# neozenith/sqlite-muninn

Measured on AMD Instinct MI355X. Metric: kNN queries/sec (10k-query batch, k=10, ef=128, 1M x 768 f32 HNSW index) + recall@10, higher is better.
Workload: dtype f32

## Files before the change

### include/muninn_hip.h

```cpp
#ifndef MUNINN_HIP_H
#define MUNINN_HIP_H

#include <stddef.h>
#include <stdint.h>

#ifdef __cplusplus
extern "C" {
#endif

#define MN_ABI_VERSION 2

typedef enum { MN_METRIC_L2 = 0, MN_METRIC_COSINE = 1, MN_METRIC_INNER_PRODUCT = 2 } mn_metric;

typedef enum { MN_ORDER_SSE = 0, MN_ORDER_WAVE = 1 } mn_order;

typedef enum {
    MN_BUILD_SEQUENTIAL = 0,
    MN_BUILD_BATCHED = 1
} mn_build_mode;

typedef struct {
    int64_t id;
    float distance;
} mn_search_result;
// ... 56 lines not shown

int mn_hnsw_slot_count(mn_index *idx);
int mn_hnsw_export_nodes(mn_index *idx, int64_t *ids, int *levels, int *deleted);
int mn_hnsw_export_vectors(mn_index *idx, float *out);
int mn_hnsw_row_width(mn_index *idx, int level);
int mn_hnsw_export_links(mn_index *idx, int level, int *out, int *width);

int64_t mn_hnsw_take_dirty(mn_index *idx, int64_t *ids, int64_t cap);

int64_t mn_hnsw_edges_of(mn_index *idx, const int64_t *ids, int n, int64_t *out_src, int64_t *out_dst, int *out_level,
                         float *out_dist, int64_t cap);

typedef struct {
    double last_kernel_ms;
    int64_t last_n_dist;
    int64_t last_n_expanded;
    int64_t last_n_overflow;
    int64_t last_n_exact_rows;
    int64_t last_n_rows_lanes4;
    int64_t last_n_rows_lanes8;
    int64_t last_n_rows_lanes16;
} mn_launch_stats;
int mn_hnsw_last_launch(mn_index *idx, mn_launch_stats *out);
typedef struct {
    double search_ms, link_ms;
    int64_t n_dist, n_expanded;
    int64_t batches, nodes;
} mn_build_stats;
int mn_hnsw_build_stats(mn_index *idx, mn_build_stats *out, int reset);
void *mn_dev_malloc(mn_index *idx, size_t bytes);
void mn_dev_free(mn_index *idx, void *p);
int mn_dev_upload(mn_index *idx, void *dst_dev, const void *src_host, size_t bytes);
int mn_dev_download(mn_index *idx, void *dst_host, const void *src_dev, size_t bytes);
int mn_hnsw_bruteforce_topk(mn_index *idx, const float *d_queries, int64_t nq, int k, int64_t *out_ids);

typedef struct {
    int64_t n_queries, n_mfma_queries, n_fallback_queries, n_rescored_rows, n_bound_violations;
    float kernel_ms;
} mn_exact_stats;
int mn_hnsw_search_exact_batch(mn_index *idx, const float *queries, int64_t nq, int k,
                               const int64_t *allow_ids, int64_t n_allow,
                               int64_t *out_ids, float *out_dists, int *out_counts);
int mn_hnsw_search_exact_batch_dev(mn_index *idx, const float *d_queries, int64_t nq, int k,
                                   const int64_t *allow_ids, int64_t n_allow,
                                   int64_t *d_out_ids, float *d_out_dists, int *d_out_counts);
int mn_hnsw_last_exact(mn_index *idx, mn_exact_stats *out);
// ... 176 lines not shown
```

### sqlite-muninn_amd/csrc/mn_beam.hpp

```cpp
#pragma once
#include "mn_dist.hpp"

template <bool COH> DEVI int ld_link(const int *p) {
    if (COH)
        return __hip_atomic_load(p, __ATOMIC_RELAXED, __HIP_MEMORY_SCOPE_AGENT);
    return *p;
}
DEVI void st_link(int *p, int v) { __hip_atomic_store(p, v, __ATOMIC_RELAXED, __HIP_MEMORY_SCOPE_AGENT); }


struct WHeap {
    uint2 *l;
    unsigned long long *g;
    int lcap, gcap;
    int size;
    int ovf;
    int sorted = 0;
};

DEVI uint2 hget(const WHeap &h, int i) {
    if (i < h.lcap)
        return h.l[i];
    unsigned long long v = __hip_atomic_load(&h.g[i - h.lcap], __ATOMIC_RELAXED, __HIP_MEMORY_SCOPE_AGENT);
    return make_uint2((unsigned)(v & 0xffffffffull), (unsigned)(v >> 32));
}
DEVI void hset(const WHeap &h, int i, uint2 v) {
    if (i < h.lcap)
        h.l[i] = v;
    else
        __hip_atomic_store(&h.g[i - h.lcap], (unsigned long long)v.x | ((unsigned long long)v.y << 32), __ATOMIC_RELAXED,
                           __HIP_MEMORY_SCOPE_AGENT);
}

DEVI void heap_push(WHeap &h, int slot, float d, int lane) {
    if (h.size + 1 >= h.lcap + h.gcap) {
        h.ovf = 1;
        return;
    }
    h.size++;
    const int idx = h.size;
    const int depth = 31 - __clz(idx);
    const bool anc = lane >= 1 && lane <= depth;
    const int p = anc ? (idx >> lane) : idx;
    const uint2 x = make_uint2(f2u(d), (unsigned)slot);
    uint2 it = x;
    if (anc)
        it = hget(h, p);
    unsigned long long stopm = __ballot(anc && (u2f(it.x) <= d));
    const int stop = stopm ? (__ffsll((long long)stopm) - 1) : depth + 1;
    if (lane >= 1 && lane < stop)
        hset(h, idx >> (lane - 1), it);
    if (lane == 0)
        hset(h, idx >> (stop - 1), x);
    __builtin_amdgcn_wave_barrier();
}

DEVI uint2 heap_pop(WHeap &h, int lane) {
    uint2 top = hget(h, 1);
    top.x = rflu(top.x);
    top.y = rflu(top.y);
    uint2 x = hget(h, h.size);
    x.x = rflu(x.x);
    x.y = rflu(x.y);
    h.size--;
    if (h.size > 0) {
        int idx = 1;
        const float xd = u2f(x.x);
        for (;;) {
            int left = 2 * idx;
            if (left > h.size)
                break;
            uint2 L, Rt;
            if (left + 1 < h.lcap) {
                uint4 c = *reinterpret_cast<const uint4 *>(&h.l[left]);
                L = make_uint2(c.x, c.y);
                Rt = make_uint2(c.z, c.w);
            } else {
                L = hget(h, left);
                Rt = (left + 1 <= h.size) ? hget(h, left + 1) : L;
            }
            L.x = rflu(L.x);
            L.y = rflu(L.y);
            Rt.x = rflu(Rt.x);
            Rt.y = rflu(Rt.y);
            int smallest = idx;
            float sd = xd;
            uint2 sv = x;
            if (u2f(L.x) < sd) {
                smallest = left;
                sd = u2f(L.x);
                sv = L;
            }
            if (left + 1 <= h.size && u2f(Rt.x) < sd) {
                smallest = left + 1;
                sv = Rt;
            }
            if (smallest == idx)
                break;
            if (lane == 0)
                hset(h, idx, sv);
            idx = smallest;
        }
        if (lane == 0)
            hset(h, idx, x);
    }
    __builtin_amdgcn_wave_barrier();
    return top;
}


struct CoopCtx {
    int *n;
    int *list;
    float *dist;
    float *qnorm;
    int nw, wv;
    float *tile = nullptr;
    int tile_rows = 0;
};

#define MN_PHASE_N 16
#ifdef MN_PHASE_TIMING
static __device__ unsigned long long mn_phase[MN_PHASE_N];
#define PH_DECL unsigned long long ph_t = __builtin_amdgcn_s_memrealtime()
#define PH_ADD(w, k)                                                                                                             \
    do {                                                                                                                         \
        const unsigned long long ph_n = __builtin_amdgcn_s_memrealtime();                                                        \
        (w).ph[k] += ph_n - ph_t;                                                                                                \
        ph_t = ph_n;                                                                                                             \
    } while (0)
#define PH_CNT(w, k, n) (w).ph[k] += (n)
#else
#define PH_DECL
#define PH_ADD(w, k)
#define PH_CNT(w, k, n)
#endif

struct WaveCtx {
#ifdef MN_PHASE_TIMING
    unsigned long long ph[MN_PHASE_N] = {0, 0, 0, 0, 0, 0, 0, 0, 0, 0, 0, 0, 0, 0, 0, 0};
#endif
    float *tile = nullptr;
    const float *q;
    float qnorm;
    int *scratch;
    unsigned long long n_dist, n_exp;
    int *rlog = nullptr;
    int rcap = 0, nr = 0;
    CoopCtx *coop = nullptr;
    int no_spec_rows = 0;
    int lp_on = 0;
    LoQuery lq = {0.0f, 0.0};
    unsigned long long n_skip = 0;
    int sv_lanes = 0;
    unsigned long long n_l8 = 0, n_l16 = 0;
};
DEVI bool getenv_spec_off(const WaveCtx &w) { return (w.no_spec_rows & 1) != 0; }

DEVI void log_row_read(const MnDevIndex &ix, WaveCtx &w, int node, int level, int lane) {
    if (!w.rlog)
        return;
    if (lane == 0 && w.nr < w.rcap) {
        int *e = w.rlog + (size_t)w.nr * MN_RLOG_INTS;
        e[0] = level == 0 ? node : -(ix.up_off[node] + level - 1) - 2;
        e[1] = (int)0xff800000u;
        e[2] = e[3] = -1;
        e[4] = 0;
    }
    w.nr++;
}
DEVI void log_greedy_detail(WaveCtx &w, float to_beat, int from, int moved_to, int lane) {
    if (!w.rlog)
        return;
    if (lane == 0 && w.nr >= 1 && w.nr <= w.rcap) {
        int *e = w.rlog + (size_t)(w.nr - 1) * MN_RLOG_INTS;
        e[1] = __float_as_int(to_beat);
        e[2] = from;
        e[3] = moved_to;
// ... 577 lines not shown
            return;
        w.n_dist = nd0;
        w.n_exp = ne0;
        w.nr = nr0;
        for (long long i = lane; i < bm_words; i += 64)
            bitmap[i] = 0u;
        __builtin_amdgcn_fence(__ATOMIC_RELEASE, "agent");
        __builtin_amdgcn_s_waitcnt(0);
        __builtin_amdgcn_wave_barrier();
    }
    res.sorted = 0;
    beam_layer<ORDER, NCH, COH, WIDE, LOG>(ix, w, cand, res, bitmap, entry, level, ef, lane);
}

DEVI uint2 res_take(WHeap &res, int i, int count, int lane) {
    if (res.sorted) {
        uint2 it = hget(res, count - i);
        it.x = rflu(it.x);
        it.y = rflu(it.y);
        return it;
    }
    return heap_pop(res, lane);
}
```

### sqlite-muninn_amd/csrc/mn_device.hpp

```cpp
#pragma once
#include <hip/hip_runtime.h>
#include <stdint.h>
#include <stdlib.h>

#define MN_WAVE 64

typedef unsigned mn_lo_t;
#define MN_LO_BITS 10
#define MN_LO_CMAX 511
#define MN_LO_LINE_CODES 96
#define MN_LO_LINE_WORDS 32
struct __align__(16) MnLoMeta {
    float scale;
    float resid;
    float xn_lo;
    float xn_hi;
};
#define MN_LO_MIN_LD 192
__host__ __device__ inline bool mn_lo_enabled(int ld) { return ld >= MN_LO_MIN_LD && (ld & 63) == 0; }
__host__ __device__ inline int mn_lo_lines(int ld) { return (ld + MN_LO_LINE_CODES - 1) / MN_LO_LINE_CODES; }
__host__ __device__ inline size_t mn_lo_row_words(int ld) { return (size_t)mn_lo_lines(ld) * MN_LO_LINE_WORDS; }
__host__ __device__ inline int mn_lo_q_floats(int ld) { return mn_lo_enabled(ld) ? mn_lo_lines(ld) * MN_LO_LINE_CODES : ld; }
__host__ __device__ inline int mn_lo_code(unsigned w, int f) { return (int)(w << (32 - MN_LO_BITS * (f + 1))) >> (32 - MN_LO_BITS); }
__host__ __device__ inline unsigned mn_lo_pack(int c0, int c1, int c2) {
// ... 3 lines not shown
constexpr int MN_ORDER_WAVE_V = 1;

struct MnDevIndex {
    const float *vectors;
    const float *norms;
    int *links0;
    int *links_up;
    const int *up_off;
    const signed char *levels;
    const unsigned char *deleted;
    unsigned char *dirty;
    const long long *ids;
    int dim, ld, metric, order;
    int W0, WU;
    int M0, MU;
    int WX;
    int n_slots;
    int n_pool_rows;
    int has_deleted;
    const mn_lo_t *vec_lo;
    const MnLoMeta *lo_meta;
};

#define MN_QC 6
struct MnSearchArgs {
    const float *queries;
    const int *query_slots;
    long long nq;
    int k;
    int ef;
    int entry_slot, max_level;
    long long *out_ids;
    float *out_dists;
    int *out_counts;
    int *sel;
    int *nsel;
    int nlev;
    const int *up_bm_index;
    unsigned *bitmap0;
    long long bm0_words;
    unsigned *bitmap_up;
    long long bmu_words;
    uint2 *cand_ovf;
    int cand_gcap;
    uint2 *res_ovf;
    int res_gcap;
    unsigned long long *counters;
    unsigned long long *q_counters;
    int use_tile;
    int lds_bitmap;
    int *readlog;
    int readcap;
    int *nread;
    int lat_tile_rows;
    unsigned lat_tile_off;
    int surv_lanes;
    int no_spec_rows;
};
size_t mn_lds_optin_limit();
bool mn_lds_grant(const void *kernel, size_t bytes);
template <typename K> inline bool mn_lds_grant_for(K kernel, size_t bytes) { return mn_lds_grant(reinterpret_cast<const void *>(kernel), bytes); }
inline int mn_no_spec_rows(long long n_slots, int ld) {
    const char *sr = getenv("MN_SPEC_ROWS");
    const bool big = (size_t)n_slots * ld * sizeof(float) > ((size_t)256 << 20);
    return sr ? (atoi(sr) == 0 ? 1 : 0) : (big ? 0 : 1);
}

#ifndef MN_CAND_LDS
#define MN_CAND_LDS 256
#endif
#ifndef MN_RES_LDS
#define MN_RES_LDS 256
#endif

void mn_module_touch_kernels();
void mn_module_touch_seq();
void mn_module_touch_spec();
void mn_module_touch_build();
void mn_launch_prep_rows(const MnDevIndex &ix, int first_slot, int n, float *norms_out, mn_lo_t *lo_out, MnLoMeta *meta_out,
                         hipStream_t st);
int mn_launch_dist_batch(int metric, int order, const float *d_query, const float *d_rows, long long n, int dim, int ld,
// ... 79 lines not shown
```

### sqlite-muninn_amd/csrc/mn_index.hip

```cpp
#include "mn_index_int.hpp"

#include <cmath>
#include <cstdarg>
#include <cstdio>
#include <unordered_map>
#include <mutex>

#define MN_MAX_M 512
#define MN_MAX_ROW 2048

static thread_local std::string g_err;

void set_err(const char *fmt, ...) {
    va_list ap;
    va_start(ap, fmt);
    mn_vformat(g_err, fmt, ap);
    va_end(ap);
}

#include <atomic>
static std::atomic<long long> g_alloc_count{0}, g_alloc_fail_at{0};
static inline void *mn_counted_alloc(size_t n) {
    const long long c = g_alloc_count.fetch_add(1, std::memory_order_relaxed) + 1;
    if (c == g_alloc_fail_at.load(std::memory_order_relaxed))
// ... 940 lines not shown
            }
            ne++;
        }
    return ne;
} MN_GUARD_END(set_err, MN_NOTHING, -1)


extern "C" int mn_hnsw_build_stats(mn_index *x, mn_build_stats *out, int reset) try {
    *out = x->bstats;
    if (reset)
        x->bstats = {0, 0, 0, 0, 0, 0};
    return 0;
} MN_GUARD_END(set_err, MN_NOTHING, -1)

extern "C" int mn_hnsw_last_launch(mn_index *x, mn_launch_stats *out) try {
    if (use_device(x))
        return -1;
    if (!x->last_on_host && fetch_counters(x))
        return -1;
    *out = x->last;
    return 0;
} MN_GUARD_END(set_err, MN_NOTHING, -1)

extern "C" void *mn_dev_malloc(mn_index *x, size_t bytes) try {
    void *p = nullptr;
    if (hipSetDevice(x->device) != hipSuccess || hipMalloc(&p, bytes) != hipSuccess) {
        set_err("mn_dev_malloc(%zu) failed", bytes);
        return nullptr;
    }
    return p;
} MN_GUARD_END(set_err, MN_NOTHING, nullptr)
extern "C" void mn_dev_free(mn_index *x, void *p) {
    (void)hipSetDevice(x->device);
    (void)hipFree(p);
}
extern "C" int mn_dev_upload(mn_index *x, void *dst, const void *src, size_t bytes) try {
    if (use_device(x))
        return -1;
    HIPCHK(hipMemcpy(dst, src, bytes, hipMemcpyHostToDevice));
    return 0;
} MN_GUARD_END(set_err, MN_NOTHING, -1)
extern "C" int mn_dev_download(mn_index *x, void *dst, const void *src, size_t bytes) try {
    if (use_device(x))
        return -1;
    HIPCHK(hipStreamSynchronize(x->stream));
    HIPCHK(hipMemcpy(dst, src, bytes, hipMemcpyDeviceToHost));
// ... 3 lines not shown
```

### sqlite-muninn_amd/csrc/mn_index_int.hpp

```cpp
#pragma once
#include "../../include/muninn_hip.h"
#include "mn_comm.hpp"
#include "mn_device.hpp"
#include "mn_guard.hpp"
#include "mn_host.hpp"

#include <algorithm>
#include <cstdlib>
#include <cstring>
#include <string>
#include <vector>

void set_err(const char *fmt, ...) __attribute__((format(printf, 1, 2)));
#define HIPCHK(expr) MN_HIPCHK(set_err, expr)

template <typename T> struct DevBuf {
    T *p = nullptr;
    size_t cap = 0;
    DevBuf() = default;
    DevBuf(const DevBuf &) = delete;
    DevBuf &operator=(const DevBuf &) = delete;
    ~DevBuf() { release(); }
    int reserve(size_t n, bool keep, hipStream_t st, int fill_byte = -1, size_t want = 0) {
        if (n <= cap)
// ... 81 lines not shown
    DevBuf<unsigned long long> ws_counters;
    DevBuf<int> ws_state;
    DevBuf<int> er_slot, er_level, er_nbr;
    DevBuf<float> er_dist;
    DevBuf<int> ws_readlog, ws_nread, ws_ncommit, d_stamp0, d_stampU, d_sidx0, d_sidxU, d_saved_rows, d_pre_act, d_pre_cnt, d_pre_row, d_spec_why;
    int spec_epoch = 0;
    std::vector<int> staged;
    DevBuf<int> d_staged;
    DevBuf<int> sh_sel, sh_nsel, sh_gcnt;
    DevBuf<int> ws_chlog;
    bool want_chlog = false;
    std::vector<int> h_chlog;
    std::vector<unsigned char> h_stale;
    int n_stale = 0;
    unsigned char *pin = nullptr;
    size_t pin_cap = 0;
    DevBuf<unsigned long long> sh_ovf;
    int sh_ovf_pending = 0;
    DevBuf<long long> sh_gids;
    DevBuf<float> sh_gd;
    long long last_spec_searched = 0;
    bool broken = false;
    mn_launch_stats last = {0, 0, 0, 0, 0, 0, 0, 0};
    mn_exact_stats last_exact = {0, 0, 0, 0, 0, 0.0f};
};

int use_device(mn_index *x);
MnDevIndex dev_view(mn_index *x);
int ht_find(const mn_index *x, int64_t id);
void ht_grow(mn_index *x);
int random_level(mn_index *x);
int host_add_node(mn_index *x, int64_t id, int level, int deleted);
int64_t first_table_full(const mn_index *x, int64_t n);
void mark_stale(mn_index *x, int slot);
struct InsertUndo {
    int first, node_count, max_level, n_pool_rows, old_cap = 0, grew_at = -1;
    unsigned rng;
    int64_t entry_id;
    std::vector<int> old_ht;
};
void undo_insert(mn_index *x, InsertUndo &u);
int sync_meta(mn_index *x);
int upload_vectors(mn_index *x, int first, const float *vecs, int n, bool src_on_device = false);
int pull_links(mn_index *x);
int push_links(mn_index *x);
unsigned char *pin_reserve(mn_index *x, size_t need);
// ... 20 lines not shown
```

### sqlite-muninn_amd/csrc/mn_index_search.hip

```cpp
#include "mn_index_int.hpp"

#include <cstdio>


static int reserve_search_ws(mn_index *x, int64_t nq, int ef) {
    hipStream_t st = x->stream;
    if (x->ws_bm0.reserve((size_t)nq * bm0_words(x->n_slots), false, st)) return -1;
    if (x->ws_cand.reserve((size_t)nq * cand_gcap(ef), false, st)) return -1;
    if (x->ws_res.reserve((size_t)nq * res_gcap(ef), false, st)) return -1;
    if (x->ws_counters.reserve(8, false, st)) return -1;
    return 0;
}

int prepare_search_ws(mn_index *x, int64_t nq, int ef, MnSearchArgs &a, bool zero_counters, bool lds_bitmap_ok) {
    hipStream_t st = x->stream;
    a.bm0_words = bm0_words(x->n_slots);
    a.cand_gcap = cand_gcap(ef);
    a.res_gcap = res_gcap(ef);
    if (reserve_search_ws(x, nq, ef))
        return -1;
    a.lds_bitmap = lds_bitmap_ok && nq <= 128 &&
                   (long long)mn_search_lds_bytes(x->ld, true) + 1024 + a.bm0_words * (long long)sizeof(unsigned) <= 64 * 1024 &&
                   !(getenv("MN_COOP") && atoi(getenv("MN_COOP")) == 0) && !(getenv("MN_LDS_BITMAP") && atoi(getenv("MN_LDS_BITMAP")) == 0);
    if (!a.lds_bitmap)
        HIPCHK(hipMemsetAsync(x->ws_bm0.p, 0, (size_t)nq * a.bm0_words * sizeof(unsigned), st));
    if (zero_counters)
        HIPCHK(hipMemsetAsync(x->ws_counters.p, 0, 8 * sizeof(unsigned long long), st));
    a.bitmap0 = x->ws_bm0.p;
    a.cand_ovf = x->ws_cand.p;
    a.res_ovf = x->ws_res.p;
    a.counters = x->ws_counters.p;
    a.bitmap_up = nullptr;
    a.bmu_words = 0;
    a.no_spec_rows = mn_no_spec_rows(x->n_slots, x->ld);
#ifdef MN_SSE_TILE_PATH
    const char *e = getenv("MN_SSE_TILE");
    a.use_tile = e ? atoi(e) : 1;
#else
    a.use_tile = 0;
#endif
    return 0;
}

void last_from_counters(mn_index *x, const unsigned long long *c, bool timed) {
    float ms = 0;
    if (!timed)
        x->last.last_kernel_ms = 0.0f;
    else if (hipEventElapsedTime(&ms, x->ev0, x->ev1) == hipSuccess)
        x->last.last_kernel_ms = ms;
    x->last.last_n_dist = (int64_t)c[0];
    x->last.last_n_expanded = (int64_t)c[1];
    x->last.last_n_overflow = (int64_t)c[2];
    x->last.last_n_exact_rows = (int64_t)(c[0] - c[3]);
    x->last.last_n_rows_lanes8 = (int64_t)c[4];
    x->last.last_n_rows_lanes16 = (int64_t)c[5];
    x->last.last_n_rows_lanes4 = x->last.last_n_exact_rows - (int64_t)(c[4] + c[5]);
}

int fetch_counters(mn_index *x) {
    unsigned long long c[8];
    if (!x->ws_counters.p)
        return 0;
    HIPCHK(hipMemcpyAsync(c, x->ws_counters.p, sizeof(c), hipMemcpyDeviceToHost, x->stream));
    HIPCHK(hipStreamSynchronize(x->stream));
    last_from_counters(x, c, true);
    return 0;
}

static int search_batch_dev_impl(mn_index *x, const float *d_queries, int64_t nq, int k, int ef, int64_t *d_ids, float *d_dists,
                                 int *d_counts, unsigned long long *q_counters) {
    if (use_device(x))
        return -1;
    if (nq <= 0)
        return 0;
    if (k <= 0) {
        set_err("mn_hnsw_search: k must be > 0");
        return -1;
    }
    if (ef < k)
        ef = k;
    hipStream_t st = x->stream;
    if (x->entry_id == -1 || x->node_count == 0) {
        HIPCHK(hipMemsetAsync(d_counts, 0, (size_t)nq * sizeof(int), st));
        HIPCHK(hipMemsetAsync(d_ids, 0xFF, (size_t)nq * k * sizeof(int64_t), st));
        HIPCHK(hipMemsetAsync(d_dists, 0, (size_t)nq * k * sizeof(float), st));
        return 0;
    }
    if (push_links(x) || sync_meta(x))
// ... 79 lines not shown
    hipStream_t st = x->stream;
    const size_t qb = (size_t)nq * x->dim * sizeof(float), ib = (size_t)nq * k * sizeof(int64_t), db = (size_t)nq * k * sizeof(float);
    const size_t cb = ((size_t)nq * sizeof(int) + 7) & ~(size_t)7;
    const size_t o_ids = (qb + 15) & ~(size_t)15, o_d = o_ids + ib, o_c = (o_d + db + 7) & ~(size_t)7, o_cnt = o_c + cb;
    const size_t need = o_cnt + (size_t)nq * MN_QC * sizeof(unsigned long long);
    if (push_links(x) || sync_meta(x))
        return -1;
    if (!pin_reserve(x, need)) {
        set_err("mn_hnsw_search: cannot allocate %zu bytes of pinned host memory", need);
        return -1;
    }
    HIPCHK(hipStreamSynchronize(st));
    memcpy(x->pin, queries, qb);
    unsigned long long *qc = reinterpret_cast<unsigned long long *>(x->pin + o_cnt);
    if (search_batch_dev_impl(x, (const float *)x->pin, nq, k, ef, (int64_t *)(x->pin + o_ids), (float *)(x->pin + o_d),
                              (int *)(x->pin + o_c), qc))
        return -1;
    const bool launched = x->entry_id != -1 && x->node_count > 0;
    HIPCHK(hipStreamSynchronize(st));
    memcpy(out_ids, x->pin + o_ids, ib);
    memcpy(out_dists, x->pin + o_d, db);
    memcpy(out_counts, x->pin + o_c, (size_t)nq * sizeof(int));
    if (launched) {
        unsigned long long tot[MN_QC] = {0, 0, 0, 0, 0, 0};
        for (int64_t q = 0; q < nq; q++)
            for (int i = 0; i < MN_QC; i++)
                tot[i] += qc[q * MN_QC + i];
        last_from_counters(x, tot, false);
        x->last_on_host = true;
        if (x->last.last_n_overflow) {
            set_err("mn_hnsw_search: %lld queries exceeded heap workspace", (long long)x->last.last_n_overflow);
            return -1;
        }
    }
    return 0;
}

template <typename F>
static int with_staged_io(mn_index *x, const float *queries, size_t nq, int k, int64_t *out_ids, float *out_dists, int *out_counts,
                          F &&dev_face) {
    hipStream_t st = x->stream;
    if (queries && x->ws_q.reserve(nq * x->dim, false, st)) return -1;
    if (x->ws_outi.reserve(nq * k, false, st)) return -1;
    if (x->ws_outd.reserve(nq * k, false, st)) return -1;
    if (x->ws_outc.reserve(nq, false, st)) return -1;
    if (queries)
        HIPCHK(hipMemcpyAsync(x->ws_q.p, queries, nq * x->dim * sizeof(float), hipMemcpyHostToDevice, st));
    if (dev_face())
        return -1;
    HIPCHK(hipMemcpyAsync(out_ids, x->ws_outi.p, nq * k * sizeof(int64_t), hipMemcpyDeviceToHost, st));
    HIPCHK(hipMemcpyAsync(out_dists, x->ws_outd.p, nq * k * sizeof(float), hipMemcpyDeviceToHost, st));
// ... 347 lines not shown
```

### sqlite-muninn_amd/csrc/mn_kernels.hip

```cpp
#include "mn_device.hpp"
#include <cstdio>
#include <cstdlib>
#include <mutex>
#include <unordered_map>

#include "mn_dist.hpp"
#include "mn_dispatch.hpp"


DEVI double wave_sum_f64(double v) {
#pragma unroll
    for (int m = 32; m >= 1; m >>= 1)
        v += __shfl_xor(v, m);
    return v;
}

template <int ORDER>
__global__ void __launch_bounds__(64)
    k_prep_rows(MnDevIndex ix, int first_slot, int n, float *norms_out, mn_lo_t *lo_out, MnLoMeta *meta_out) {
    extern __shared__ float lds[];
    const int lane = threadIdx.x;
    int slot = first_slot + blockIdx.x;
    if (blockIdx.x >= n)
        return;
    const float *row = ix.vectors + (size_t)slot * ix.ld;
// ... 191 lines not shown
        w.lq.qs_lo = rfl_f64(w.lq.qs_lo);
        w.lq.qn_hi = rfl_f64(w.lq.qn_hi);
        w.qnorm = u2f(rflu(f2u(w.qnorm)));
        w.sv_lanes = a.surv_lanes;
    }
    if (BUILD && a.readlog) {
        w.rlog = a.readlog + (size_t)qi * a.readcap * MN_RLOG_INTS;
        w.rcap = a.readcap;
    }

    WHeap cand, res;
    cand.l = cand_l;
    cand.lcap = MN_CAND_LDS;
    cand.g = reinterpret_cast<unsigned long long *>(a.cand_ovf + (size_t)qi * a.cand_gcap);
    cand.gcap = a.cand_gcap;
    cand.size = 0;
    cand.ovf = 0;
    res.l = res_l;
    res.lcap = MN_RES_LDS;
    res.g = reinterpret_cast<unsigned long long *>(a.res_ovf + (size_t)qi * a.res_gcap);
    res.gcap = a.res_gcap;
    res.size = 0;
    res.ovf = 0;

    unsigned *bm0 = lds_bitmap ? lds_bitmap : a.bitmap0 + (size_t)qi * a.bm0_words;
    int cur = a.entry_slot;

    if (!BUILD) {
        for (int l = a.max_level; l > 0; l--)
            cur = greedy_layer<ORDER, NCH, false, WIDE>(ix, w, cur, l, lane);
        if (LAT)
            beam_layer_auto<ORDER, NCH, false, WIDE>(ix, w, cand, res, bm0, a.bm0_words, cur, 0, a.ef, lane);
        else
            beam_layer<ORDER, NCH, false, WIDE, false, LP>(ix, w, cand, res, bm0, cur, 0, a.ef, lane);
        int count = res.size;
        int outn = count < a.k ? count : a.k;
        for (int i = count - 1; i >= 0; i--) {
            uint2 it = res_take(res, i, count, lane);
            if (i < a.k && lane == 0) {
                a.out_ids[qi * a.k + i] = ix.ids[it.y];
                a.out_dists[qi * a.k + i] = -u2f(it.x);
            }
        }
        if (lane == 0) {
            for (int i = outn; i < a.k; i++) {
                a.out_ids[qi * a.k + i] = -1;
                a.out_dists[qi * a.k + i] = 0.0f;
            }
            a.out_counts[qi] = outn;
        }
    } else {
        const int level = ix.levels[qslot];
        for (int l = a.max_level; l > level; l--)
            cur = greedy_layer<ORDER, NCH, false, WIDE, LAT>(ix, w, cur, l, lane);
        int start = level < a.max_level ? level : a.max_level;
        for (int l = start; l >= 0; l--) {
            unsigned *bm = bm0;
            if (l > 0)
                bm = a.bitmap_up + ((size_t)a.up_bm_index[qi] * a.max_level + (l - 1)) * a.bmu_words;
            if (LAT)
                beam_layer_auto<ORDER, NCH, false, WIDE, true>(ix, w, cand, res, bm, l > 0 ? a.bmu_words : a.bm0_words, cur, l, a.ef, lane);
            else
                beam_layer<ORDER, NCH, false, WIDE>(ix, w, cand, res, bm, cur, l, a.ef, lane);
            const int M_max = (l == 0) ? ix.M0 : ix.MU;
            int count = res.size;
            int keep = count < M_max ? count : M_max;
            int *sel = a.sel + ((size_t)qi * a.nlev + l) * ix.M0;
            int first = cur;
            for (int i = count - 1; i >= 0; i--) {
                uint2 it = res_take(res, i, count, lane);
                if (i < keep && lane == 0)
                    sel[i] = (int)it.y;
                if (i == 0)
                    first = (int)it.y;
            }
            if (lane == 0)
                a.nsel[qi * a.nlev + l] = keep;
            if (count > 0)
                cur = first;
        }
    }
    if (lane == 0) {
        if (BUILD && a.readlog)
            a.nread[qi] = LAT ? w.nr : a.readcap + 1;
        if (a.q_counters) {
            a.q_counters[(size_t)qi * MN_QC + 0] = w.n_dist;
            a.q_counters[(size_t)qi * MN_QC + 1] = w.n_exp;
            a.q_counters[(size_t)qi * MN_QC + 2] = (cand.ovf || res.ovf) ? 1ull : 0ull;
            a.q_counters[(size_t)qi * MN_QC + 3] = w.n_skip;
            a.q_counters[(size_t)qi * MN_QC + 4] = w.n_l8;
            a.q_counters[(size_t)qi * MN_QC + 5] = w.n_l16;
        } else {
            atomicAdd(&a.counters[0], w.n_dist);
            atomicAdd(&a.counters[1], w.n_exp);
            if (cand.ovf || res.ovf)
                atomicAdd(&a.counters[2], 1ull);
            if (LP && w.n_skip)
                atomicAdd(&a.counters[3], w.n_skip);
            if (LP && w.n_l8)
                atomicAdd(&a.counters[4], w.n_l8);
            if (LP && w.n_l16)
                atomicAdd(&a.counters[5], w.n_l16);
        }
    }
}

template <int ORDER, int NCH, bool BUILD, bool WIDE = false, bool LP = false>
__global__ void __launch_bounds__(64) k_beam(MnDevIndex ix, MnSearchArgs a) {
    extern __shared__ __align__(16) unsigned char smem[];
    if ((long long)blockIdx.x >= a.nq)
        return;
    beam_query<ORDER, NCH, BUILD, WIDE, false, LP>(ix, a, blockIdx.x, threadIdx.x, smem, nullptr);
}

#define MN_COOP_WAVES 8
// ... 132 lines not shown
    const char *lp = getenv("MN_LOWPREC_FILTER");
    if (!build && ix.vec_lo && ix.lo_meta && !(lp && atoi(lp) == 0)) {
        MnSearchArgs al = a;
        const char *sv = getenv("MN_SURVIVOR_LANES");
        const int svl = sv ? atoi(sv) : 0;
        al.surv_lanes = (svl == 4 || svl == 8 || svl == 16) ? svl : 0;
        if (wide)
            hipLaunchKernelGGL((k_beam<ORDER, NCH, false, true, true>), grid, block, lds, st, ix, al);
        else
            hipLaunchKernelGGL((k_beam<ORDER, NCH, false, false, true>), grid, block, lds, st, ix, al);
        return;
    }
    if (wide) {
        if (build)
            hipLaunchKernelGGL((k_beam<ORDER, NCH, true, true>), grid, block, lds, st, ix, a);
        else
            hipLaunchKernelGGL((k_beam<ORDER, NCH, false, true>), grid, block, lds, st, ix, a);
    } else if (build)
        hipLaunchKernelGGL((k_beam<ORDER, NCH, true>), grid, block, lds, st, ix, a);
    else
        hipLaunchKernelGGL((k_beam<ORDER, NCH, false>), grid, block, lds, st, ix, a);
}

int mn_launch_search(const MnDevIndex &ix, const MnSearchArgs &a, bool build, hipStream_t st) {
    if (a.nq <= 0)
        return 0;
    if (ix.order == MN_ORDER_SSE_V) {
        const char *qe = getenv("MN_SSE_QUAD");
        if (MN_SSE_QUAD2 > 0 && (ix.dim >> 4) >= MN_SSE_QUAD2 && !(qe && atoi(qe) == 0))
            launch_beam<MN_ORDER_SSE_V, 1>(ix, a, build, st);
        else
            launch_beam<MN_ORDER_SSE_V, 0>(ix, a, build, st);
        return 0;
    }
    mn_for_wave_walk(ix.ld, [&](auto O, auto N) { launch_beam<O(), N()>(ix, a, build, st); });
    return 0;
}


template <int ORDER, int NCH>
__global__ void __launch_bounds__(64)
    k_edge_rows(MnDevIndex ix, const int *row_slot, const int *row_level, int n_rows, int *out_nbr, float *out_dist) {
    extern __shared__ __align__(16) unsigned char smem[];
    const int lane = threadIdx.x;
    const int r = blockIdx.x;
    if (r >= n_rows)
        return;
    float *q = reinterpret_cast<float *>(smem);
    const int s = row_slot[r], level = row_level[r];
// ... 96 lines not shown
```

### sqlite-muninn_amd/csrc/mn_seq.hip

```cpp
#include "mn_beam.hpp"
#include "mn_prune.hpp"
#include "mn_dispatch.hpp"

struct MnSeqArgs {
    const int *slots;
    int n;
    int ef;
    int *state;
    unsigned *bitmap0;
    long long bm0_words;
    unsigned *bitmap_up;
    long long bmu_words;
    uint2 *cand_ovf;
    int cand_gcap;
    uint2 *res_ovf;
    int res_gcap;
    unsigned long long *counters;
    int SB;
    int LW;
    int *chlog;
    int chcap;
    int pre_rows, pre_w;
    int wave_floats, lat_tile_rows;
    int no_spec_rows;
};
#define MN_CH_INTS 5

DEVI void seq_log(const MnSeqArgs &a, int &nlog, int op, int src, int level, int dst, unsigned dist_bits) {
    if (nlog < 0)
        return;
    if (nlog >= a.chcap) {
        nlog = -1;
        return;
    }
    int *e = a.chlog + 1 + (size_t)nlog * MN_CH_INTS;
    e[0] = op;
    e[1] = src;
    e[2] = level;
    e[3] = dst;
    e[4] = (int)dist_bits;
    nlog++;
}

DEVI int *seq_row(const MnDevIndex &ix, int node, int level) {
    if (level == 0)
        return ix.links0 + (size_t)node * ix.W0;
    return ix.links_up + ((size_t)ix.up_off[node] + (level - 1)) * ix.WU;
// ... 93 lines not shown
    if (coop.wv != 0) {
        seq_helper<ORDER, NCH>(ix, a, q, coop, selbuf, pre_nd, pre_cnt, tvw, lane);
        return;
    }

    WaveCtx w;
    w.coop = &coop;
    w.no_spec_rows = a.no_spec_rows;
    w.q = q;
    w.scratch = scratch;
    w.n_dist = 0;
    w.n_exp = 0;
    WHeap cand, res;
    cand.l = cand_l;
    cand.lcap = MN_CAND_LDS;
    cand.g = reinterpret_cast<unsigned long long *>(a.cand_ovf);
    cand.gcap = a.cand_gcap;
    cand.size = 0;
    cand.ovf = 0;
    res.l = res_l;
    res.lcap = MN_RES_LDS;
    res.g = reinterpret_cast<unsigned long long *>(a.res_ovf);
    res.gcap = a.res_gcap;
    res.size = 0;
    res.ovf = 0;

    int entry = a.state[0];
    int maxl = a.state[1];
    int nlog = a.chlog ? 0 : -1;

    for (int it = 0; it < a.n; it++) {
        const int s = a.slots[it];
        const int level = ix.levels[s];
        const float *sv = ix.vectors + (size_t)s * ix.ld;
        __builtin_amdgcn_wave_barrier();
        for (int i = lane; i < ix.ld; i += 64)
            q[i] = sv[i];
        __builtin_amdgcn_s_waitcnt(0);
        __builtin_amdgcn_wave_barrier();
        w.qnorm = ix.metric == 1 ? ix.norms[s] : 0.0f;
        if (lane == 0)
            *coop.qnorm = w.qnorm;

        int cur = entry;
        for (int l = maxl; l > level; l--)
            cur = greedy_layer<ORDER, NCH, true, WIDE>(ix, w, cur, l, lane);
// ... 170 lines not shown
    a.state = d_state;
    a.bitmap0 = bitmap0;
    a.bm0_words = bm0_words;
    a.bitmap_up = bitmap_up;
    a.bmu_words = bmu_words;
    a.cand_ovf = cand_ovf;
    a.cand_gcap = cand_gcap;
    a.res_ovf = res_ovf;
    a.res_gcap = res_gcap;
    a.counters = counters;
    a.SB = (ix.M0 + 63) & ~63;
    a.LW = (ix.WX + 1 + 63) & ~63;
    if (a.LW < 192)
        a.LW = 192;
    size_t lds = mn_insert_seq_lds_bytes(ix);
    const size_t base = lds - MN_SEQ_COOP_BYTES;
    int pre_rows = 0, pre_w = 0;
    size_t pre = seq_pre_bytes(ix, &pre_rows, &pre_w);
    const char *pe = getenv("MN_SEQ_PRE");
    if (pe && atoi(pe) == 0)
        pre = 0;
    a.pre_rows = a.pre_w = a.wave_floats = a.lat_tile_rows = 0;
    a.no_spec_rows = mn_no_spec_rows(ix.n_slots, ix.ld);
    const size_t lds0 = lds;
    const char *te = getenv("MN_LAT_TILE");
    for (int rows = ix.order == MN_ORDER_SSE_V && ix.ld >= 256 && !(te && atoi(te) == 0) ? 4 : 0; rows >= 0; rows = rows == 4 ? 2 : rows == 2 ? 0 : -1) {
        const int wf = std::max(pre ? ix.ld : 0, rows ? mn_lat_tile_floats(ix.ld, rows) : 0);
        const size_t need = lds0 + pre + (size_t)MN_SEQ_WAVES * wf * sizeof(float);
        if (rows == 0 && !pre)
            break;
        if (need <= (rows ? mn_lds_optin_limit() : (size_t)MN_LDS_LIMIT)) {
            lds = need;
            a.wave_floats = wf;
            a.lat_tile_rows = rows;
            if (pre) {
                a.pre_rows = pre_rows;
                a.pre_w = pre_w;
            }
            break;
        }
    }
    const char *co = getenv("MN_COOP");
    const dim3 blk(co && atoi(co) == 0 ? 64 : MN_SEQ_WAVES * 64);
    mn_for_row_walk(ix.order, ix.ld, [&](auto O, auto N) {
        if (lds > 64 * 1024) {
            const void *kp = ix.WX > 64 ? reinterpret_cast<const void *>(k_insert_seq<O(), N(), true>)
// ... 40 lines not shown
```

### sqlite-muninn_amd/hnsw.py

```python
from __future__ import annotations

import ctypes as C
import os

import numpy as np

from .build import LIB

METRIC = {"l2": 0, "cosine": 1, "inner_product": 2}
ORDER_SSE, ORDER_WAVE = 0, 1
BUILD_SEQUENTIAL, BUILD_BATCHED = 0, 1

_f32p = np.ctypeslib.ndpointer(np.float32, flags="C_CONTIGUOUS")
_i64p = np.ctypeslib.ndpointer(np.int64, flags="C_CONTIGUOUS")
_i32p = np.ctypeslib.ndpointer(np.int32, flags="C_CONTIGUOUS")


class MuninnHipError(RuntimeError):
    pass


class _Result(C.Structure):
    _fields_ = [("id", C.c_int64), ("distance", C.c_float)]

# ... 63 lines not shown
    ("mn_hnsw_delete", C.c_int, [C.c_void_p, C.c_int64]),
    ("mn_hnsw_get_vector", C.c_int, [C.c_void_p, C.c_int64, _f32p]),
    ("mn_hnsw_node_count", C.c_int, [C.c_void_p]),
    ("mn_hnsw_entry_point", C.c_int64, [C.c_void_p]),
    ("mn_hnsw_max_level", C.c_int, [C.c_void_p]),
    ("mn_hnsw_node_level", C.c_int, [C.c_void_p, C.c_int64]),
    ("mn_hnsw_node_deleted", C.c_int, [C.c_void_p, C.c_int64]),
    ("mn_hnsw_neighbors", C.c_int, [C.c_void_p, C.c_int64, C.c_int, _i64p, C.c_int]),
    ("mn_hnsw_load_node", C.c_int, [C.c_void_p, C.c_int64, _f32p, C.c_int, C.c_int]),
    ("mn_hnsw_load_neighbors", C.c_int, [C.c_void_p, C.c_int64, C.c_int, _i64p, C.c_int]),
    ("mn_hnsw_set_entry", C.c_int, [C.c_void_p, C.c_int64, C.c_int]),
    ("mn_hnsw_slot_count", C.c_int, [C.c_void_p]),
    ("mn_hnsw_export_nodes", C.c_int, [C.c_void_p, _i64p, _i32p, _i32p]),
    ("mn_hnsw_export_vectors", C.c_int, [C.c_void_p, _f32p]),
    ("mn_hnsw_export_links", C.c_int, [C.c_void_p, C.c_int, _i32p, C.POINTER(C.c_int)]),
    ("mn_hnsw_row_width", C.c_int, [C.c_void_p, C.c_int]),
    ("mn_hnsw_batch_stage", C.c_int, [C.c_void_p, _i64p, _f32p, C.c_int64]),
    ("mn_hnsw_batch_dims", C.c_int, [C.c_void_p, C.POINTER(C.c_int), C.POINTER(C.c_int)]),
    ("mn_hnsw_batch_search", C.c_int, [C.c_void_p, C.c_int, C.c_int, C.c_void_p, C.c_void_p]),
    ("mn_hnsw_batch_link", C.c_int, [C.c_void_p, C.c_void_p, C.c_void_p]),
    ("mn_hnsw_take_dirty", C.c_int64, [C.c_void_p, _i64p, C.c_int64]),
    ("mn_hnsw_edges_of", C.c_int64, [C.c_void_p, _i64p, C.c_int, _i64p, _i64p, _i32p, _f32p, C.c_int64]),
    ("mn_hnsw_last_launch", C.c_int, [C.c_void_p, C.POINTER(LaunchStats)]),
    ("mn_hnsw_build_stats", C.c_int, [C.c_void_p, C.POINTER(BuildStats), C.c_int]),
    ("mn_dev_malloc", C.c_void_p, [C.c_void_p, C.c_size_t]),
    ("mn_dev_free", None, [C.c_void_p, C.c_void_p]),
    ("mn_dev_upload", C.c_int, [C.c_void_p, C.c_void_p, C.c_void_p, C.c_size_t]),
    ("mn_dev_download", C.c_int, [C.c_void_p, C.c_void_p, C.c_void_p, C.c_size_t]),
    ("mn_hnsw_bruteforce_topk", C.c_int, [C.c_void_p, C.c_void_p, C.c_int64, C.c_int, _i64p]),
    ("mn_hnsw_search_exact_batch", C.c_int,
     [C.c_void_p, _f32p, C.c_int64, C.c_int, C.c_void_p, C.c_int64, _i64p, _f32p, _i32p]),
    ("mn_hnsw_search_exact_batch_dev", C.c_int,
     [C.c_void_p, C.c_void_p, C.c_int64, C.c_int, C.c_void_p, C.c_int64, C.c_void_p, C.c_void_p, C.c_void_p]),
    ("mn_hnsw_last_exact", C.c_int, [C.c_void_p, C.POINTER(ExactStats)]),
    ("mn_hnsw_knn_graph", C.c_int, [C.c_void_p, C.c_int, C.c_float, _i64p, _f32p, _i32p]),
    ("mn_hnsw_knn_graph_dev", C.c_int, [C.c_void_p, C.c_int, C.c_float, C.c_void_p, C.c_void_p, C.c_void_p]),
    ("mn_comm_unique_id", C.c_int, [C.c_void_p]),
    ("mn_comm_init_rccl", C.c_void_p, [C.c_int, C.c_int, C.c_void_p, C.c_int]),
    ("mn_comm_init_host", C.c_void_p, [C.c_int, C.c_int, C.c_void_p, C.c_void_p, C.c_int]),
    ("mn_comm_world", C.c_int, [C.c_void_p]),
    ("mn_comm_rank", C.c_int, [C.c_void_p]),
    ("mn_comm_destroy", None, [C.c_void_p]),
    ("mn_comm_last_error", C.c_char_p, []),
    ("mn_hnsw_build_shared", C.c_int, [C.c_void_p, C.c_void_p, _i64p, _f32p, C.c_int64, C.c_int, C.c_int, C.c_int]),
    ("mn_hnsw_search_sharded_dev", C.c_int, [C.c_void_p, C.c_void_p, C.c_void_p, C.c_int64, C.c_int, C.c_int, C.c_void_p,
                                             C.c_void_p, C.c_void_p]),
# ... 352 lines not shown
            cap = int(n)

    def edges_of(self, ids):
        ids = np.ascontiguousarray(ids, np.int64)
        cap = max(64, len(ids) * 4 * self.M)
        while True:
            src = np.empty(cap, np.int64)
            dst = np.empty(cap, np.int64)
            lvl = np.empty(cap, np.int32)
            dist = np.empty(cap, np.float32)
            n = self.L.mn_hnsw_edges_of(self.h, ids, len(ids), src, dst, lvl, dist, cap)
            if n < 0:
                raise MuninnHipError(_err())
            if n <= cap:
                return src[:n], dst[:n], lvl[:n], dist[:n]
            cap = n

    def last_launch(self):
        s = LaunchStats()
        if self.L.mn_hnsw_last_launch(self.h, C.byref(s)) != 0:
            raise MuninnHipError(_err())
        return {n: getattr(s, n) for n, _ in LaunchStats._fields_}

    def build_stats(self, reset=False):
        s = BuildStats()
        self.L.mn_hnsw_build_stats(self.h, C.byref(s), 1 if reset else 0)
        return {n: getattr(s, n) for n, _ in BuildStats._fields_}

    def dev_malloc(self, nbytes):
        p = self.L.mn_dev_malloc(self.h, nbytes)
        if not p:
            raise MuninnHipError(_err())
        return p

    def dev_free(self, p):
        self.L.mn_dev_free(self.h, p)

    def dev_upload(self, dptr, arr):
        arr = np.ascontiguousarray(arr)
        if self.L.mn_dev_upload(self.h, dptr, arr.ctypes.data, arr.nbytes) != 0:
            raise MuninnHipError(_err())

    def dev_download(self, arr, dptr):
        if self.L.mn_dev_download(self.h, arr.ctypes.data, dptr, arr.nbytes) != 0:
            raise MuninnHipError(_err())

# ... 14 lines not shown
```

Before: 597,400.

## Parallelize heap pop sift-down path and drain result heap by rank

Heap pop no longer walks the sift-down serially. It ballots child comparisons across the wave to precompute the min-child path, then places the moved element with a single wave-parallel shift, and falls back to the serial loop for large or global-overflow heaps or NaN keys. The final result drain replaces repeated heap pops with a rank-based parallel placement in which each lane counts the keys greater than its own. It also adds heap counters, env flags to restore the old behavior, and a stats API. The costs are an O(count^2) rank loop and more per-pop LDS reads.

```diff
diff --git a/include/muninn_hip.h b/include/muninn_hip.h
--- a/include/muninn_hip.h
+++ b/include/muninn_hip.h
@@ -102,6 +102,7 @@
     int64_t last_n_rows_lanes16;
 } mn_launch_stats;
 int mn_hnsw_last_launch(mn_index *idx, mn_launch_stats *out);
+int mn_hnsw_last_heap_stats(mn_index *idx, int64_t out[4]);
 typedef struct {
     double search_ms, link_ms;
     int64_t n_dist, n_expanded;
diff --git a/sqlite-muninn_amd/csrc/mn_beam.hpp b/sqlite-muninn_amd/csrc/mn_beam.hpp
--- a/sqlite-muninn_amd/csrc/mn_beam.hpp
+++ b/sqlite-muninn_amd/csrc/mn_beam.hpp
@@ -16,6 +16,8 @@
     int size;
     int ovf;
     int sorted = 0;
+    int serial = 0;
+    unsigned n_path = 0, n_loop = 0;
 };
 
 DEVI uint2 hget(const WHeap &h, int i) {
@@ -55,6 +57,47 @@
     __builtin_amdgcn_wave_barrier();
 }
 
+DEVI void sift_down_from(WHeap &h, int idx, uint2 x, int lane) {
+    const float xd = u2f(x.x);
+    for (;;) {
+        int left = 2 * idx;
+        if (left > h.size)
+            break;
+        uint2 L, Rt;
+        if (left + 1 < h.lcap) {
+            uint4 c = *reinterpret_cast<const uint4 *>(&h.l[left]);
+            L = make_uint2(c.x, c.y);
+            Rt = make_uint2(c.z, c.w);
+        } else {
+            L = hget(h, left);
+            Rt = (left + 1 <= h.size) ? hget(h, left + 1) : L;
+        }
+        L.x = rflu(L.x);
+        L.y = rflu(L.y);
+        Rt.x = rflu(Rt.x);
+        Rt.y = rflu(Rt.y);
+        int smallest = idx;
+        float sd = xd;
+        uint2 sv = x;
+        if (u2f(L.x) < sd) {
+            smallest = left;
+            sd = u2f(L.x);
+            sv = L;
+        }
+        if (left + 1 <= h.size && u2f(Rt.x) < sd) {
+            smallest = left + 1;
+            sv = Rt;
+        }
+        if (smallest == idx)
+            break;
+        if (lane == 0)
+            hset(h, idx, sv);
+        idx = smallest;
+    }
+    if (lane == 0)
+        hset(h, idx, x);
+}
+
 DEVI uint2 heap_pop(WHeap &h, int lane) {
     uint2 top = hget(h, 1);
     top.x = rflu(top.x);
@@ -63,46 +106,69 @@
     x.x = rflu(x.x);
     x.y = rflu(x.y);
     h.size--;
-    if (h.size > 0) {
-        int idx = 1;
+    const int n = h.size;
+    if (n > 0) {
+        const int in_lds = (h.lcap - 2) >> 1;
+        const int nint = (n >> 1) < in_lds ? (n >> 1) : in_lds;
         const float xd = u2f(x.x);
-        for (;;) {
-            int left = 2 * idx;
-            if (left > h.size)
-                break;
-            uint2 L, Rt;
-            if (left + 1 < h.lcap) {
-                uint4 c = *reinterpret_cast<const uint4 *>(&h.l[left]);
-                L = make_uint2(c.x, c.y);
-                Rt = make_uint2(c.z, c.w);
-            } else {
-                L = hget(h, left);
-                Rt = (left + 1 <= h.size) ? hget(h, left + 1) : L;
-            }
-            L.x = rflu(L.x);
-            L.y = rflu(L.y);
-            Rt.x = rflu(Rt.x);
-            Rt.y = rflu(Rt.y);
-            int smallest = idx;
-            float sd = xd;
-            uint2 sv = x;
-            if (u2f(L.x) < sd) {
-                smallest = left;
-                sd = u2f(L.x);
-                sv = L;
-            }
-            if (left + 1 <= h.size && u2f(Rt.x) < sd) {
-                smallest = left + 1;
-                sv = Rt;
-            }
-            if (smallest == idx)
-                break;
-            if (lane == 0)
-                hset(h, idx, sv);
-            idx = smallest;
-        }
-        if (lane == 0)
-            hset(h, idx, x);
+        bool nan = !(xd == xd);
+        unsigned long long m0 = 0ull, m1 = 0ull, m2 = 0ull, m3 = 0ull;
+        int hl = lane;
+        asm volatile("" : "+v"(hl));
+        const bool by_loop = h.serial || nint > 256;
+        if (!by_loop) {
+#pragma unroll 1
+            for (int t = 0; t * 64 < nint; t++) {
+                const int i = 1 + t * 64 + hl;
+                const bool in = i <= nint;
+                const bool has_r = in && 2 * i + 1 <= n;
+                float kl = 0.0f, kr = 0.0f;
+                if (in) {
+                    kl = u2f(h.l[2 * i].x);
+                    kr = u2f(h.l[2 * i + 1].x);
+                }
+                nan = nan || (in && !(kl == kl)) || (has_r && !(kr == kr));
+                const unsigned long long m = __ballot(has_r && kr < kl);
+                m0 = t == 0 ? m : m0;
+                m1 = t == 1 ? m : m1;
+                m2 = t == 2 ? m : m2;
+                m3 = t == 3 ? m : m3;
+            }
+        }
+        int from = 1;
+        if (!by_loop && !__ballot(nan)) {
+            int p = 1, k = 0;
+            while (p <= nint) {
+                const int b = p - 1;
+                const unsigned long long m = b < 64 ? m0 : b < 128 ? m1 : b < 192 ? m2 : m3;
+                p = 2 * p + (int)((m >> (b & 63)) & 1ull);
+                k++;
+            }
+            const bool on = hl >= 1 && hl <= k;
+            const int mypos = on ? p >> (k - hl) : 1;
+            uint2 it = x;
+            if (on)
+                it = h.l[mypos];
+            const unsigned long long stopm = __ballot(on && !(u2f(it.x) < xd));
+            const int stop = stopm ? (__ffsll((long long)stopm) - 1) : k + 1;
+            if (hl >= 1 && hl < stop)
+                h.l[mypos >> 1] = it;
+            from = 0;
+            if (stop <= k) {
+                if (hl == stop)
+                    h.l[mypos >> 1] = x;
+            } else if (2 * p <= n) {
+                from = p;
+            } else if (hl == 0) {
+                hset(h, p, x);
+            }
+        }
+        if (from) {
+            h.n_loop++;
+            sift_down_from(h, from, x, lane);
+        } else {
+            h.n_path++;
+        }
     }
     __builtin_amdgcn_wave_barrier();
     return top;
@@ -119,7 +185,7 @@
     int tile_rows = 0;
 };
 
-#define MN_PHASE_N 16
+#define MN_PHASE_N 18
 #ifdef MN_PHASE_TIMING
 static __device__ unsigned long long mn_phase[MN_PHASE_N];
 #define PH_DECL unsigned long long ph_t = __builtin_amdgcn_s_memrealtime()
@@ -138,7 +204,7 @@
 
 struct WaveCtx {
 #ifdef MN_PHASE_TIMING
-    unsigned long long ph[MN_PHASE_N] = {0, 0, 0, 0, 0, 0, 0, 0, 0, 0, 0, 0, 0, 0, 0, 0};
+    unsigned long long ph[MN_PHASE_N] = {0, 0, 0, 0, 0, 0, 0, 0, 0, 0, 0, 0, 0, 0, 0, 0, 0, 0};
 #endif
     float *tile = nullptr;
     const float *q;
@@ -154,6 +220,7 @@
     unsigned long long n_skip = 0;
     int sv_lanes = 0;
     unsigned long long n_l8 = 0, n_l16 = 0;
+    unsigned n_drain_rank = 0, n_drain_pops = 0;
 };
 DEVI bool getenv_spec_off(const WaveCtx &w) { return (w.no_spec_rows & 1) != 0; }
 
@@ -777,3 +844,31 @@
     }
     return heap_pop(res, lane);
 }
+
+DEVI bool res_rank_drain(WHeap &res, uint2 *perm, int count, int want, int lane) {
+    if (res.sorted || count < 1 || count >= res.lcap)
+        return false;
+    bool bad = false;
+#pragma unroll 1
+    for (int t0 = 0; t0 < count; t0 += 64) {
+        const bool have = t0 + lane < count;
+        uint2 it = make_uint2(0u, 0u);
+        if (have)
+            it = res.l[t0 + lane + 1];
+        const float key = have ? u2f(it.x) : __builtin_nanf("");
+        int above = 0, below = 0;
+        for (int m = 1; m <= count; m++) {
+            const float km = u2f(res.l[m].x);
+            above += km > key ? 1 : 0;
+            below += km < key ? 1 : 0;
+        }
+        bad = bad || (have && above + below != count - 1);
+        if (have && above < want)
+            perm[above] = it;
+    }
+    if (__ballot(bad))
+        return false;
+    res.size = 0;
+    __builtin_amdgcn_wave_barrier();
+    return true;
+}
diff --git a/sqlite-muninn_amd/csrc/mn_device.hpp b/sqlite-muninn_amd/csrc/mn_device.hpp
--- a/sqlite-muninn_amd/csrc/mn_device.hpp
+++ b/sqlite-muninn_amd/csrc/mn_device.hpp
@@ -49,7 +49,10 @@
     const MnLoMeta *lo_meta;
 };
 
-#define MN_QC 6
+#define MN_QC 10
+#define MN_NCOUNTERS 12
+#define MN_HEAP_POP_SERIAL 1
+#define MN_HEAP_DRAIN_POPS 2
 struct MnSearchArgs {
     const float *queries;
     const int *query_slots;
@@ -83,7 +86,9 @@
     unsigned lat_tile_off;
     int surv_lanes;
     int no_spec_rows;
+    int heap_flags;
 };
+int mn_heap_flags_from_env();
 size_t mn_lds_optin_limit();
 bool mn_lds_grant(const void *kernel, size_t bytes);
 template <typename K> inline bool mn_lds_grant_for(K kernel, size_t bytes) { return mn_lds_grant(reinterpret_cast<const void *>(kernel), bytes); }
diff --git a/sqlite-muninn_amd/csrc/mn_index.hip b/sqlite-muninn_amd/csrc/mn_index.hip
--- a/sqlite-muninn_amd/csrc/mn_index.hip
+++ b/sqlite-muninn_amd/csrc/mn_index.hip
@@ -986,6 +986,16 @@
     return 0;
 } MN_GUARD_END(set_err, MN_NOTHING, -1)
 
+extern "C" int mn_hnsw_last_heap_stats(mn_index *x, int64_t out[4]) try {
+    if (use_device(x))
+        return -1;
+    if (!x->last_on_host && fetch_counters(x))
+        return -1;
+    for (int i = 0; i < 4; i++)
+        out[i] = x->last_heap[i];
+    return 0;
+} MN_GUARD_END(set_err, MN_NOTHING, -1)
+
 extern "C" void *mn_dev_malloc(mn_index *x, size_t bytes) try {
     void *p = nullptr;
     if (hipSetDevice(x->device) != hipSuccess || hipMalloc(&p, bytes) != hipSuccess) {
diff --git a/sqlite-muninn_amd/csrc/mn_index_int.hpp b/sqlite-muninn_amd/csrc/mn_index_int.hpp
--- a/sqlite-muninn_amd/csrc/mn_index_int.hpp
+++ b/sqlite-muninn_amd/csrc/mn_index_int.hpp
@@ -127,6 +127,7 @@
     long long last_spec_searched = 0;
     bool broken = false;
     mn_launch_stats last = {0, 0, 0, 0, 0, 0, 0, 0};
+    int64_t last_heap[4] = {0, 0, 0, 0};
     mn_exact_stats last_exact = {0, 0, 0, 0, 0, 0.0f};
 };
 
diff --git a/sqlite-muninn_amd/csrc/mn_index_search.hip b/sqlite-muninn_amd/csrc/mn_index_search.hip
--- a/sqlite-muninn_amd/csrc/mn_index_search.hip
+++ b/sqlite-muninn_amd/csrc/mn_index_search.hip
@@ -8,7 +8,7 @@
     if (x->ws_bm0.reserve((size_t)nq * bm0_words(x->n_slots), false, st)) return -1;
     if (x->ws_cand.reserve((size_t)nq * cand_gcap(ef), false, st)) return -1;
     if (x->ws_res.reserve((size_t)nq * res_gcap(ef), false, st)) return -1;
-    if (x->ws_counters.reserve(8, false, st)) return -1;
+    if (x->ws_counters.reserve(MN_NCOUNTERS, false, st)) return -1;
     return 0;
 }
 
@@ -25,7 +25,7 @@
     if (!a.lds_bitmap)
         HIPCHK(hipMemsetAsync(x->ws_bm0.p, 0, (size_t)nq * a.bm0_words * sizeof(unsigned), st));
     if (zero_counters)
-        HIPCHK(hipMemsetAsync(x->ws_counters.p, 0, 8 * sizeof(unsigned long long), st));
+        HIPCHK(hipMemsetAsync(x->ws_counters.p, 0, MN_NCOUNTERS * sizeof(unsigned long long), st));
     a.bitmap0 = x->ws_bm0.p;
     a.cand_ovf = x->ws_cand.p;
     a.res_ovf = x->ws_res.p;
@@ -58,12 +58,14 @@
 }
 
 int fetch_counters(mn_index *x) {
-    unsigned long long c[8];
+    unsigned long long c[MN_NCOUNTERS];
     if (!x->ws_counters.p)
         return 0;
     HIPCHK(hipMemcpyAsync(c, x->ws_counters.p, sizeof(c), hipMemcpyDeviceToHost, x->stream));
     HIPCHK(hipStreamSynchronize(x->stream));
     last_from_counters(x, c, true);
+    for (int i = 0; i < 4; i++)
+        x->last_heap[i] = (int64_t)c[6 + i];
     return 0;
 }
 
@@ -189,11 +191,13 @@
     memcpy(out_dists, x->pin + o_d, db);
     memcpy(out_counts, x->pin + o_c, (size_t)nq * sizeof(int));
     if (launched) {
-        unsigned long long tot[MN_QC] = {0, 0, 0, 0, 0, 0};
+        unsigned long long tot[MN_QC] = {0};
         for (int64_t q = 0; q < nq; q++)
             for (int i = 0; i < MN_QC; i++)
                 tot[i] += qc[q * MN_QC + i];
         last_from_counters(x, tot, false);
+        for (int i = 0; i < 4; i++)
+            x->last_heap[i] = (int64_t)tot[6 + i];
         x->last_on_host = true;
         if (x->last.last_n_overflow) {
             set_err("mn_hnsw_search: %lld queries exceeded heap workspace", (long long)x->last.last_n_overflow);
diff --git a/sqlite-muninn_amd/csrc/mn_kernels.hip b/sqlite-muninn_amd/csrc/mn_kernels.hip
--- a/sqlite-muninn_amd/csrc/mn_kernels.hip
+++ b/sqlite-muninn_amd/csrc/mn_kernels.hip
@@ -1,6 +1,7 @@
 #include "mn_device.hpp"
 #include <cstdio>
 #include <cstdlib>
+#include <cstring>
 #include <mutex>
 #include <unordered_map>
 
@@ -238,6 +239,8 @@
     res.gcap = a.res_gcap;
     res.size = 0;
     res.ovf = 0;
+    cand.serial = res.serial = (a.heap_flags & MN_HEAP_POP_SERIAL) ? 1 : 0;
+    const bool drain_by_rank = !(a.heap_flags & MN_HEAP_DRAIN_POPS);
 
     unsigned *bm0 = lds_bitmap ? lds_bitmap : a.bitmap0 + (size_t)qi * a.bm0_words;
     int cur = a.entry_slot;
@@ -251,13 +254,33 @@
             beam_layer<ORDER, NCH, false, WIDE, false, LP>(ix, w, cand, res, bm0, cur, 0, a.ef, lane);
         int count = res.size;
         int outn = count < a.k ? count : a.k;
-        for (int i = count - 1; i >= 0; i--) {
-            uint2 it = res_take(res, i, count, lane);
-            if (i < a.k && lane == 0) {
+        PH_DECL;
+        if (drain_by_rank && res_rank_drain(res, cand.l, count, a.k, lane)) {
+            w.n_drain_rank++;
+            for (int i = lane; i < outn; i += 64) {
+                const uint2 it = cand.l[i];
                 a.out_ids[qi * a.k + i] = ix.ids[it.y];
                 a.out_dists[qi * a.k + i] = -u2f(it.x);
             }
-        }
+        } else {
+            if (count > 0 && !res.sorted)
+                w.n_drain_pops++;
+            for (int i = count - 1; i >= 0; i--) {
+                uint2 it = res_take(res, i, count, lane);
+                if (i < a.k && lane == 0) {
+                    a.out_ids[qi * a.k + i] = ix.ids[it.y];
+                    a.out_dists[qi * a.k + i] = -u2f(it.x);
+                }
+            }
+        }
+        PH_ADD(w, 16);
+        PH_CNT(w, 17, 1);
+#ifdef MN_PHASE_TIMING
+        if (lane == 0) {
+            atomicAdd(&mn_phase[16], w.ph[16]);
+            atomicAdd(&mn_phase[17], w.ph[17]);
+        }
+#endif
         if (lane == 0) {
             for (int i = outn; i < a.k; i++) {
                 a.out_ids[qi * a.k + i] = -1;
@@ -283,12 +306,22 @@
             int keep = count < M_max ? count : M_max;
             int *sel = a.sel + ((size_t)qi * a.nlev + l) * ix.M0;
             int first = cur;
-            for (int i = count - 1; i >= 0; i--) {
-                uint2 it = res_take(res, i, count, lane);
-                if (i < keep && lane == 0)
-                    sel[i] = (int)it.y;
-                if (i == 0)
-                    first = (int)it.y;
+            if (drain_by_rank && res_rank_drain(res, cand.l, count, keep > 1 ? keep : 1, lane)) {
+                w.n_drain_rank++;
+                for (int i = lane; i < keep; i += 64)
+                    sel[i] = (int)cand.l[i].y;
+                first = (int)rflu(cand.l[0].y);
+                __builtin_amdgcn_wave_barrier();
+            } else {
+                if (count > 0 && !res.sorted)
+                    w.n_drain_pops++;
+                for (int i = count - 1; i >= 0; i--) {
+                    uint2 it = res_take(res, i, count, lane);
+                    if (i < keep && lane == 0)
+                        sel[i] = (int)it.y;
+                    if (i == 0)
+                        first = (int)it.y;
+                }
             }
             if (lane == 0)
                 a.nsel[qi * a.nlev + l] = keep;
@@ -306,7 +339,19 @@
             a.q_counters[(size_t)qi * MN_QC + 3] = w.n_skip;
             a.q_counters[(size_t)qi * MN_QC + 4] = w.n_l8;
             a.q_counters[(size_t)qi * MN_QC + 5] = w.n_l16;
+            a.q_counters[(size_t)qi * MN_QC + 6] = (unsigned long long)cand.n_path + res.n_path;
+            a.q_counters[(size_t)qi * MN_QC + 7] = (unsigned long long)cand.n_loop + res.n_loop;
+            a.q_counters[(size_t)qi * MN_QC + 8] = w.n_drain_rank;
+            a.q_counters[(size_t)qi * MN_QC + 9] = w.n_drain_pops;
         } else {
+            if (cand.n_path + res.n_path)
+                atomicAdd(&a.counters[6], (unsigned long long)cand.n_path + res.n_path);
+            if (cand.n_loop + res.n_loop)
+                atomicAdd(&a.counters[7], (unsigned long long)cand.n_loop + res.n_loop);
+            if (w.n_drain_rank)
+                atomicAdd(&a.counters[8], (unsigned long long)w.n_drain_rank);
+            if (w.n_drain_pops)
+                atomicAdd(&a.counters[9], (unsigned long long)w.n_drain_pops);
             atomicAdd(&a.counters[0], w.n_dist);
             atomicAdd(&a.counters[1], w.n_exp);
             if (cand.ovf || res.ovf)
@@ -485,9 +530,22 @@
         hipLaunchKernelGGL((k_beam<ORDER, NCH, false>), grid, block, lds, st, ix, a);
 }
 
-int mn_launch_search(const MnDevIndex &ix, const MnSearchArgs &a, bool build, hipStream_t st) {
-    if (a.nq <= 0)
+int mn_heap_flags_from_env() {
+    int f = 0;
+    const char *e = getenv("MN_HEAP_POP");
+    if (e && !strcmp(e, "serial"))
+        f |= MN_HEAP_POP_SERIAL;
+    e = getenv("MN_DRAIN");
+    if (e && !strcmp(e, "pops"))
+        f |= MN_HEAP_DRAIN_POPS;
+    return f;
+}
+
+int mn_launch_search(const MnDevIndex &ix, const MnSearchArgs &a_in, bool build, hipStream_t st) {
+    if (a_in.nq <= 0)
         return 0;
+    MnSearchArgs a = a_in;
+    a.heap_flags = mn_heap_flags_from_env();
     if (ix.order == MN_ORDER_SSE_V) {
         const char *qe = getenv("MN_SSE_QUAD");
         if (MN_SSE_QUAD2 > 0 && (ix.dim >> 4) >= MN_SSE_QUAD2 && !(qe && atoi(qe) == 0))
diff --git a/sqlite-muninn_amd/csrc/mn_seq.hip b/sqlite-muninn_amd/csrc/mn_seq.hip
--- a/sqlite-muninn_amd/csrc/mn_seq.hip
+++ b/sqlite-muninn_amd/csrc/mn_seq.hip
@@ -23,6 +23,7 @@
     int pre_rows, pre_w;
     int wave_floats, lat_tile_rows;
     int no_spec_rows;
+    int heap_serial;
 };
 #define MN_CH_INTS 5
 
@@ -162,6 +163,7 @@
     res.lcap = MN_RES_LDS;
     res.g = reinterpret_cast<unsigned long long *>(a.res_ovf);
     res.gcap = a.res_gcap;
+    cand.serial = res.serial = a.heap_serial;
     res.size = 0;
     res.ovf = 0;
 
@@ -378,6 +380,7 @@
         pre = 0;
     a.pre_rows = a.pre_w = a.wave_floats = a.lat_tile_rows = 0;
     a.no_spec_rows = mn_no_spec_rows(ix.n_slots, ix.ld);
+    a.heap_serial = (mn_heap_flags_from_env() & MN_HEAP_POP_SERIAL) ? 1 : 0;
     const size_t lds0 = lds;
     const char *te = getenv("MN_LAT_TILE");
     for (int rows = ix.order == MN_ORDER_SSE_V && ix.ld >= 256 && !(te && atoi(te) == 0) ? 4 : 0; rows >= 0; rows = rows == 4 ? 2 : rows == 2 ? 0 : -1) {
diff --git a/sqlite-muninn_amd/hnsw.py b/sqlite-muninn_amd/hnsw.py
--- a/sqlite-muninn_amd/hnsw.py
+++ b/sqlite-muninn_amd/hnsw.py
@@ -109,6 +109,7 @@
     ("mn_hnsw_take_dirty", C.c_int64, [C.c_void_p, _i64p, C.c_int64]),
     ("mn_hnsw_edges_of", C.c_int64, [C.c_void_p, _i64p, C.c_int, _i64p, _i64p, _i32p, _f32p, C.c_int64]),
     ("mn_hnsw_last_launch", C.c_int, [C.c_void_p, C.POINTER(LaunchStats)]),
+    ("mn_hnsw_last_heap_stats", C.c_int, [C.c_void_p, C.POINTER(C.c_int64)]),
     ("mn_hnsw_build_stats", C.c_int, [C.c_void_p, C.POINTER(BuildStats), C.c_int]),
     ("mn_dev_malloc", C.c_void_p, [C.c_void_p, C.c_size_t]),
     ("mn_dev_free", None, [C.c_void_p, C.c_void_p]),
@@ -507,6 +508,12 @@
             raise MuninnHipError(_err())
         return {n: getattr(s, n) for n, _ in LaunchStats._fields_}
 
+    def last_heap_stats(self):
+        a = (C.c_int64 * 4)()
+        if self.L.mn_hnsw_last_heap_stats(self.h, a) != 0:
+            raise MuninnHipError(_err())
+        return tuple(int(v) for v in a)
+
     def build_stats(self, reset=False):
         s = BuildStats()
         self.L.mn_hnsw_build_stats(self.h, C.byref(s), 1 if reset else 0)
```

Measured after the change: 626,300 (median of 6 runs). +4.8%, better.
